# amikey/kaldi-ctc

Hardware: AMD Instinct MI355X
Metric: CTC-train frames/sec, 5×BLSTM-512 mb=16, at 1/2/4/8 MI355X; loss match (higher is better)
Workload: dtype f32

## Files before the change

include/ctc.h:

```cpp
#ifndef KALDI_CTC_AMD_CTC_H_
#define KALDI_CTC_AMD_CTC_H_

#include <stddef.h>

#ifdef __cplusplus
extern "C" {
#endif

struct ihipStream_t;
typedef struct ihipStream_t *ctcStream_t;

typedef enum {
  CTC_STATUS_SUCCESS = 0,
  CTC_STATUS_MEMOPS_FAILED = 1,
  CTC_STATUS_INVALID_VALUE = 2,
  CTC_STATUS_EXECUTION_FAILED = 3,
  CTC_STATUS_UNKNOWN_ERROR = 4
} ctcStatus_t;

typedef enum { CTC_CPU = 0, CTC_GPU = 1 } ctcComputeLocation;

struct ctcOptions {
  ctcComputeLocation loc;
  union {
// ... 11 lines not shown
                             const int *const input_lengths, int alphabet_size,
                             int minibatch, float *costs, void *workspace,
                             struct ctcOptions options);

ctcStatus_t get_workspace_size(const int *const label_lengths,
                               const int *const input_lengths, int alphabet_size,
                               int minibatch, struct ctcOptions info,
                               size_t *size_bytes);

ctcStatus_t mictc_compute_ctc_loss_async(const float *activations, float *gradients,
                                         const int *flat_labels, const int *label_lengths,
                                         const int *input_lengths, int alphabet_size,
                                         int minibatch, double *costs_dev, void *workspace,
                                         ctcStream_t stream, int blank_label);

int mictc_set_frame_group(int m);

int mictc_set_win(int on);

#ifdef __cplusplus
}
#endif
#endif
```

kaldi-ctc_amd/csrc/ctc.hip:

```cpp
#include <algorithm>
#include <cstring>
#include <type_traits>
#include <atomic>
#include <vector>

#include "common.h"
#include "ctc.h"
#include "prof.h"

namespace kctc {
namespace ctcimpl {

constexpr int kMaxLabel = 639;
constexpr int kThreads = 256;
constexpr int kABThreads = 512;
constexpr int kABWaves = kABThreads / 64;
constexpr int kSPT = (2 * kMaxLabel + 1 + kABThreads - 1) / kABThreads;
constexpr int kFR = 8;

struct UttDesc {
  int T, L, S, feasible, lab_off, pad;
  long long ab_off;
  long long off_off;
};
// ... 478 lines not shown
}

template <bool SPILL, int SPT>
__global__ __launch_bounds__(kABThreads) void ctc_alpha_beta(
    const float *__restrict__ lp, int N, int A, int blank, UttDesc *__restrict__ descs,
    const int *__restrict__ labels, float *__restrict__ spill, double *__restrict__ offs,
    double *__restrict__ costs, AbLds lay) {
  if (blockIdx.x >= (unsigned)N) ab_body<SPILL, SPT, true>(lp, N, A, blank, descs, labels, spill, offs, costs, lay);
  else ab_body<SPILL, SPT, false>(lp, N, A, blank, descs, labels, spill, offs, costs, lay);
}

__global__ __launch_bounds__(kThreads) void ctc_grad(
    const float *__restrict__ acts, const float *__restrict__ logz, float *__restrict__ grads,
    int N, int A, int T_max, int blank, const UttDesc *__restrict__ descs,
    const int *__restrict__ links, const int *__restrict__ owners, const float *__restrict__ spill,
    const double *__restrict__ offs, const double *__restrict__ costs) {
  extern __shared__ __attribute__((aligned(16))) char smem[];
  const int n = blockIdx.y, t0 = blockIdx.x * kFR, tid = threadIdx.x;
  const UttDesc d = descs[n];
  const int T = d.feasible ? d.T : 0, L = d.L, S = d.S;
  const int nf = min(kFR, T_max - t0);
  if (t0 >= T) {
    for (int it = tid; it < nf * A; it += kThreads) {
      int f = it / A, a = it - f * A;
      grads[((long)(t0 + f) * N + n) * A + a] = 0.f;
    }
    return;
  }
  float *occ = reinterpret_cast<float *>(smem);
  int *nxt = reinterpret_cast<int *>(occ + kFR * S);
  int *owner = nxt + (L > 0 ? L : 1);
  float *gblank = reinterpret_cast<float *>(owner + A);
  float *gtot = gblank + kFR;
  for (int a = tid; a < A; a += kThreads) owner[a] = owners[(long)n * A + a];
  for (int j = tid; j < L; j += kThreads) nxt[j] = links[d.lab_off + j];
  const double logp = -costs[n];
  const float *al = spill + d.ab_off;
  const float *be = al + (long long)T * S;
  const double *oa = offs + d.off_off, *ob = oa + T;
  const int nreal = min(nf, T - t0);
// ... 22 lines not shown
  __syncthreads();
  for (int it = tid; it < nf * A; it += kThreads) {
    const int f = it / A, a = it - f * A, t = t0 + f;
    const long idx = ((long)t * N + n) * A + a;
    float g = 0.f;
    if (t < T) {
      float gam = 0.f;
      if (a == blank) {
        gam = gblank[f];
      } else {
        for (int j = owner[a]; j >= 0; j = nxt[j]) gam += occ[f * S + 2 * j + 1];
        gam *= gtot[f];
      }
      g = expf(acts[idx] - logz[(long)t * N + n]) - gam;
    }
    grads[idx] = g;
  }
}

struct Staging {
  char *buf = nullptr;
  size_t cap = 0;
  hipEvent_t ev = nullptr;
  bool pending = false;
};
static thread_local Staging g_stage;

static char *staging_acquire(size_t bytes) {
  Staging &s = g_stage;
  if (s.pending) {
    if (hipEventSynchronize(s.ev) != hipSuccess) return nullptr;
// ... 18 lines not shown
static std::atomic<int> g_frame_group{0};
static int frame_group() {
  int m = g_frame_group.load(std::memory_order_relaxed);
  if (m <= 0) {
    m = 8;
    int expect = 0;
    g_frame_group.compare_exchange_strong(expect, m);
    m = g_frame_group.load(std::memory_order_relaxed);
  }
  return m;
}

static std::atomic<int> g_win{1};
static bool win_enabled() { return g_win.load(std::memory_order_relaxed) != 0; }

static ctcStatus_t launch(const float *acts, float *grads, const int *flat_labels,
                          const int *label_lengths, const int *input_lengths, int A, int N,
                          double *costs_dev, void *workspace, hipStream_t stream, int blank) {
  Layout lay;
  std::vector<UttDesc> descs;
  bool bad = false;
  if (!make_layout(label_lengths, input_lengths, A, N, &lay, &descs, &bad) || bad)
    return CTC_STATUS_INVALID_VALUE;
  if (blank < 0 || blank >= A || !acts || !workspace) return CTC_STATUS_INVALID_VALUE;
  long long nlab = 0;
  for (int n = 0; n < N; n++) nlab += label_lengths[n];
  for (long long i = 0; i < nlab; i++)
    if (flat_labels[i] < 0 || flat_labels[i] >= A || flat_labels[i] == blank)
      return CTC_STATUS_INVALID_VALUE;
  char *ws = static_cast<char *>(workspace);
  char *stage = staging_acquire(lay.costs);
  if (!stage) return CTC_STATUS_MEMOPS_FAILED;
  memcpy(stage + lay.desc, descs.data(), sizeof(UttDesc) * N);
  if (nlab) memcpy(stage + lay.labels, flat_labels, sizeof(int) * nlab);
  {
    int *links = reinterpret_cast<int *>(stage + lay.links), *owner = reinterpret_cast<int *>(stage + lay.owner);
    std::fill(owner, owner + (size_t)N * A, -1);
    long long off = 0;
    for (int n = 0; n < N; n++) {
      const int L = label_lengths[n];
      int *own = owner + (size_t)n * A;
      for (int j = L - 1; j >= 0; j--) {
        const int k = flat_labels[off + j];
        links[off + j] = own[k];
        own[k] = j;
      }
      off += L;
    }
  }
  if (hipMemcpyAsync(ws, stage, lay.costs, hipMemcpyHostToDevice, stream) != hipSuccess)
    return CTC_STATUS_MEMOPS_FAILED;
  staging_release(stream);
  UttDesc *d_desc = reinterpret_cast<UttDesc *>(ws + lay.desc);
  const int *d_lab = reinterpret_cast<const int *>(ws + lay.labels);
  float *d_logz = reinterpret_cast<float *>(ws + lay.logz);
  float *d_spill = reinterpret_cast<float *>(ws + lay.spill);
  double *d_offs = reinterpret_cast<double *>(ws + lay.offs);
  const long rows = (long)lay.T_max * N;
  float *d_lp = reinterpret_cast<float *>(ws + lay.lp);
  if (rows > 0) {
    ProfSpan ps(stream, "ctc_logz");
    hipLaunchKernelGGL(ctc_logz, dim3(ceil_div(rows, 4)), dim3(256), 0, stream, acts, A, rows,
                       d_logz, d_lp);
  }
  const int want = grads != nullptr;
  {
    int Smax = 1;
// ... 34 lines not shown
        else go(ctc_alpha_beta<false, kSPT>, N);
      }
    }
  }
  if (want && lay.T_max > 0) {
    int Lmax = 0;
    for (int n = 0; n < N; n++) Lmax = label_lengths[n] > Lmax ? label_lengths[n] : Lmax;
    const int Smax = 2 * Lmax + 1;
    size_t shm = sizeof(float) * kFR * Smax + sizeof(int) * (Lmax > 0 ? Lmax : 1) +
                 sizeof(int) * A + 2 * sizeof(float) * kFR;
    if (shm > 160 * 1024) return CTC_STATUS_INVALID_VALUE;
    ProfSpan ps(stream, "ctc_grad");
    hipLaunchKernelGGL(ctc_grad, dim3(ceil_div(lay.T_max, kFR), N), dim3(kThreads), shm, stream,
                       acts, d_logz, grads, N, A, lay.T_max, blank, d_desc,
                       reinterpret_cast<const int *>(ws + lay.links), reinterpret_cast<const int *>(ws + lay.owner),
                       d_spill, d_offs, costs_dev);
  }
  if (hipGetLastError() != hipSuccess) return CTC_STATUS_EXECUTION_FAILED;
  return CTC_STATUS_SUCCESS;
}

}
}

using namespace kctc::ctcimpl;

extern "C" {

int get_warpctc_version(void) { return 2; }

int mictc_set_frame_group(int m) {
// ... 26 lines not shown
  Layout lay;
  bool bad = false;
  if (!make_layout(label_lengths, input_lengths, alphabet_size, minibatch, &lay, nullptr, &bad) ||
      bad)
    return CTC_STATUS_INVALID_VALUE;
  *size_bytes = lay.total;
  return CTC_STATUS_SUCCESS;
}

ctcStatus_t mictc_compute_ctc_loss_async(const float *activations, float *gradients,
                                         const int *flat_labels, const int *label_lengths,
                                         const int *input_lengths, int alphabet_size,
                                         int minibatch, double *costs_dev, void *workspace,
                                         ctcStream_t stream, int blank_label) {
  if (!costs_dev) return CTC_STATUS_INVALID_VALUE;
  try {
    return launch(activations, gradients, flat_labels, label_lengths, input_lengths,
                  alphabet_size, minibatch, costs_dev, workspace,
                  reinterpret_cast<hipStream_t>(stream), blank_label);
  } catch (...) {
    return CTC_STATUS_UNKNOWN_ERROR;
  }
}

ctcStatus_t compute_ctc_loss(const float *const activations, float *gradients,
                             const int *const flat_labels, const int *const label_lengths,
                             const int *const input_lengths, int alphabet_size, int minibatch,
                             float *costs, void *workspace, struct ctcOptions options) {
  if (options.loc != CTC_GPU || !costs) return CTC_STATUS_INVALID_VALUE;
  Layout lay;
  bool bad = false;
  if (!make_layout(label_lengths, input_lengths, alphabet_size, minibatch, &lay, nullptr, &bad) ||
      bad)
    return CTC_STATUS_INVALID_VALUE;
// ... 18 lines not shown
```

kaldi-ctc_amd/csrc/elementwise.h:

```cpp
#pragma once
#include <hip/hip_runtime.h>

#include <cstddef>

namespace kctc {

void clip_sgd_update(hipStream_t s, float *w, const float *dw, long n, float lr, float clip,
                     const unsigned *skip = nullptr);
void momentum_update(hipStream_t s, float *w, float *delta, const float *dw, long n, float lr, float clip,
                     float m, const unsigned *skip = nullptr);
void rownorm_clip(hipStream_t s, float *d, long rows, int dim, float thr, int *nclipped);
void row_argmax(hipStream_t s, const float *m, long rows, int cols, int *ids);
size_t sum_rows_ws_floats(long rows, int cols);
void sum_rows(hipStream_t s, const float *X, long rows, int cols, float alpha, float beta,
              float *out, float *ws);
void fill(hipStream_t s, float *p, long n, float v);
void scale_inplace(hipStream_t s, float *p, long n, float alpha);
void axpy(hipStream_t s, float *y, const float *x, long n, float alpha);
void add_randn(hipStream_t s, float *x, long n, float stddev, unsigned long long seed);
size_t dot_ws_bytes();
void dot_f64(hipStream_t s, const float *a, const float *b, long n, double *out, void *ws);

constexpr int kMaxSplice = 32;
void splice_rows(hipStream_t s, const float *in, int dim, int ns, long rows, const int *ctx, int nctx, int first,
// ... 15 lines not shown
```

kaldi-ctc_amd/csrc/elementwise.hip:

```cpp
#include "common.h"
#include "elementwise.h"

namespace kctc {
namespace {

typedef float floatx4 __attribute__((ext_vector_type(4)));

__global__ __launch_bounds__(256) void k_clip_sgd(float *__restrict__ w, const float *__restrict__ dw,
                                                  long n, float lr, float clip, const unsigned *skip) {
  if (skip && *skip) return;
  const long n4 = n / 4;
  const long stride = (long)gridDim.x * 256;
  const bool vec = ((uintptr_t)w % 16 == 0) && ((uintptr_t)dw % 16 == 0);
  long i = (long)blockIdx.x * 256 + threadIdx.x;
  if (vec) {
    for (; i < n4; i += stride) {
      floatx4 g = reinterpret_cast<const floatx4 *>(dw)[i];
      floatx4 v = reinterpret_cast<floatx4 *>(w)[i];
#pragma unroll
      for (int j = 0; j < 4; j++) {
        float x = g[j];
        if (clip > 0.f) x = fminf(fmaxf(x, -clip), clip);
        v[j] += lr * x;
      }
      reinterpret_cast<floatx4 *>(w)[i] = v;
    }
    i = n4 * 4 + (long)blockIdx.x * 256 + threadIdx.x;
  }
  for (; i < n; i += stride) {
    float x = dw[i];
    if (clip > 0.f) x = fminf(fmaxf(x, -clip), clip);
    w[i] += lr * x;
  }
}

__global__ __launch_bounds__(256) void k_rownorm_clip(float *__restrict__ d, long rows, int dim,
                                                      float inv_thr2, int *__restrict__ nclipped) {
  const long row = (long)blockIdx.x * 4 + (threadIdx.x >> 6);
  const int lane = threadIdx.x & 63;
  __shared__ int cnt[4];
  int clipped = 0;
  if (row < rows) {
    float *r = d + row * dim;
    float ss = 0.f;
    const bool vec = (dim % 4 == 0) && ((uintptr_t)r % 16 == 0);
    if (vec) {
      for (int j = lane; j < dim / 4; j += 64) {
        floatx4 v = reinterpret_cast<const floatx4 *>(r)[j];
// ... 109 lines not shown
  }
}

void momentum_update(hipStream_t s, float *w, float *delta, const float *dw, long n, float lr, float clip,
                     float m, const unsigned *skip) {
  if (n <= 0) return;
  hipLaunchKernelGGL(k_momentum, dim3(grid_for(n)), dim3(256), 0, s, w, delta, dw, n, lr, clip, m, skip);
}

void clip_sgd_update(hipStream_t s, float *w, const float *dw, long n, float lr, float clip,
                     const unsigned *skip) {
  if (n <= 0) return;
  hipLaunchKernelGGL(k_clip_sgd, dim3(grid_for((n + 3) / 4)), dim3(256), 0, s, w, dw, n, lr, clip, skip);
}

void rownorm_clip(hipStream_t s, float *d, long rows, int dim, float thr, int *nclipped) {
  if (rows <= 0) return;
  hipLaunchKernelGGL(k_rownorm_clip, dim3(ceil_div(rows, 4)), dim3(256), 0, s, d, rows, dim,
                     1.f / (thr * thr), nclipped);
}

void row_argmax(hipStream_t s, const float *m, long rows, int cols, int *ids) {
  if (rows <= 0) return;
  hipLaunchKernelGGL(k_row_argmax, dim3(ceil_div(rows, 4)), dim3(256), 0, s, m, rows, cols, ids);
}

size_t sum_rows_ws_floats(long rows, int cols) { return (size_t)64 * cols; }

void sum_rows(hipStream_t s, const float *X, long rows, int cols, float alpha, float beta,
              float *out, float *ws) {
// ... 197 lines not shown
```

kaldi-ctc_amd/csrc/nnet.cpp:

```cpp
#include "nnet.h"
#include "kaldi_io.h"

#include <algorithm>
#include <cmath>
#include <cstdio>
#include <cstring>
#include <iomanip>
#include <iostream>
#include <sstream>

#include "common.h"
#include "ctc.h"
#include "decodable.h"
#include "dropout.h"
#include "elementwise.h"
#include "gemm.h"
#include "prof.h"

namespace kctc {
namespace nnet2 {

int levenshtein(const int *ref, int m, const int *hyp, int n) {
  if (m <= 0) return n > 0 ? n : 0;
  if (n <= 0) return m;
// ... 136 lines not shown

uint64_t Rng::next() {
  uint64_t z = (s += 0x9E3779B97F4A7C15ULL);
  z = (z ^ (z >> 30)) * 0xBF58476D1CE4E5B9ULL;
  z = (z ^ (z >> 27)) * 0x94D049BB133111EBULL;
  return z ^ (z >> 31);
}
double Rng::uniform() { return ((double)(next() >> 11) + 0.5) * (1.0 / 9007199254740992.0); }
double Rng::gauss() {
  const double u1 = uniform(), u2 = uniform();
  return std::sqrt(-2.0 * std::log(u1)) * std::cos(6.283185307179586 * u2);
}

static hipStream_t S() { return CuDevice::Instantiate().stream; }

static std::vector<std::string> split_ws(const std::string &s) {
  std::vector<std::string> out;
  std::istringstream is(s);
  std::string t;
  while (is >> t) out.push_back(t);
  return out;
}

static bool take(const std::string &name, std::string *args, std::string *val) {
  auto parts = split_ws(*args);
  const std::string ne = name + "=";
  for (size_t i = 0; i < parts.size(); i++) {
    if (parts[i].compare(0, ne.size(), ne) == 0) {
      *val = parts[i].substr(ne.size());
      std::string rest;
// ... 339 lines not shown
                                 workspace_.p, workspace_.bytes, reserve_.p, reserve_.bytes, DeviceError(),
                                 dev0.stream2, &wg);
      if (st) throw std::runtime_error("rnn_backward_data failed: " + std::to_string(st));
    }
    if (!wg.done) {
      dev0.Fork();
      ProfScope ps("layer_rnn_backward_weights", ws);
      int st = rnn_backward_weights(desc_, ws, T, N, in_value.Data(), out_value.Data(), workspace_.p,
                                    workspace_.bytes, to_update->grad_.f(), reserve_.p, reserve_.bytes,
                                    side_gemm_blocks(), input_bound_, nullptr, packed_input_cols(T, N), false,
                                    wgrad_prepack(in_value, out_value));
      if (st) throw std::runtime_error("rnn_backward_weights failed: " + std::to_string(st));
    }
    return;
  }
  {
    ProfScope ps("layer_rnn_backward_data");
    const RnnPrepack *pre = pre_.done && pre_ver_ == pver_ ? &pre_ : nullptr;
    int st = rnn_backward_data(desc_, S(), T, N, out_value.Data(), out_deriv.Data(), params_.f(),
                               in_deriv ? in_deriv->Data() : nullptr, workspace_.p, workspace_.bytes,
                               reserve_.p, reserve_.bytes, DeviceError(), CuDevice::Instantiate().stream2, nullptr,
                               pre);
    if (st) throw std::runtime_error("rnn_backward_data failed: " + std::to_string(st));
  }
  if (to_update_in) {
    auto *to_update = dynamic_cast<CuDNNRecurrentComponent *>(to_update_in);
    if (!to_update) throw std::invalid_argument("CuDNNRecurrentComponent: bad to_update");
    auto &dev = CuDevice::Instantiate();
    hipStream_t ws = dev.side ? dev.side : S();
    dev.Fork();
    to_update->grad_stream_ = ws;
    KCTC_HIP_CHECK(hipMemsetAsync(to_update->grad_.p, 0, sizeof(float) * NumParameters(), ws));
    ProfScope ps("layer_rnn_backward_weights", ws);
    int st = rnn_backward_weights(desc_, ws, T, N, in_value.Data(), out_value.Data(), workspace_.p,
                                  workspace_.bytes, to_update->grad_.f(), reserve_.p, reserve_.bytes,
                                  dev.side ? side_gemm_blocks() : 0, input_bound_,
                                  (!in_deriv && dev.side) ? dev.stream2 : nullptr, packed_input_cols(T, N),
                                  in_deriv && dev.side,
                                  wgrad_prepack(in_value, out_value));
    if (st) throw std::runtime_error("rnn_backward_weights failed: " + std::to_string(st));
  }
}

const RnnPrepack *CuDNNRecurrentComponent::wgrad_prepack(const CuMatrixBase &in_value,
                                                         const CuMatrixBase &out_value) const {
  return pre_.wdone && in_value.Data() == pre_x_ && out_value.Data() == pre_y_ ? &pre_ : nullptr;
}

bool CuDNNRecurrentComponent::PackedOutput(const void **rows, const void **cols) const {
  *rows = *cols = nullptr;
  if (!reserve_.p || seq_length_ <= 0 || mini_batch_ <= 0) return false;
  if (reserve_.bytes < sizeof(float) * (size_t)rnn_reserve_layout(desc_, seq_length_, mini_batch_).total) return false;
// ... 65 lines not shown

void UpdatableComponent::Scale(float scale) { scale_inplace(S(), ParamData(), NumParameters(), scale); }

void UpdatableComponent::Add(float alpha, const UpdatableComponent &other) {
  CheckSameKind(other, "Add");
  axpy(S(), ParamData(), const_cast<UpdatableComponent &>(other).ParamData(), NumParameters(), alpha);
}

int CuDNNRecurrentComponent::side_gemm_blocks() const {
  return 512;
}

void CuDNNRecurrentComponent::ApplyUpdate(const unsigned *skip) {
  ++pver_;
  UpdateWith(params_.f(), grad_.f(), clip_gradient_, skip);
}

Component *CuDNNRecurrentComponent::Copy() const {
  auto *c = new CuDNNRecurrentComponent;
  c->CopyUpdatableFrom(*this);
  c->desc_ = desc_;
  c->max_seq_length_ = max_seq_length_;
  c->param_stddev_ = param_stddev_;
  c->bias_stddev_ = bias_stddev_;
  c->clip_gradient_ = clip_gradient_;
  const long P = NumParameters();
  c->params_.ensure(sizeof(float) * P);
  c->grad_.ensure(sizeof(float) * P);
  KCTC_HIP_CHECK(hipMemcpyAsync(c->params_.p, params_.p, sizeof(float) * P, hipMemcpyDeviceToDevice, S()));
  return c;
// ... 505 lines not shown
    gemm_f32(S(), g);
  }
  if (to_update_in) {
    auto *to_update = dynamic_cast<AffineComponent *>(to_update_in);
    if (!to_update) throw std::invalid_argument("AffineComponent: bad to_update");
    GemmArgs g;
    g.transA = true;
    g.M = out_dim_; g.N = in_dim_; g.K = (int)rows;
    g.A = out_deriv.Data(); g.lda = out_dim_;
    g.B = in_value.Data(); g.ldb = in_dim_;
    g.C = to_update->grad_.f(); g.ldc = in_dim_;
    g.split_k = gemm_pick_split(g.M, g.N, g.K, 1);
    const size_t wsf = (size_t)g.split_k * g.M * g.N + sum_rows_ws_floats(rows, out_dim_);
    ws_.ensure(sizeof(float) * wsf);
    g.ws = ws_.f();
    gemm_f32(S(), g);
    sum_rows(S(), out_deriv.Data(), rows, out_dim_, 1.f, 0.f,
             to_update->grad_.f() + (long)in_dim_ * out_dim_, ws_.f() + (size_t)g.split_k * g.M * g.N);
  }
}

Component *AffineComponent::Copy() const {
  auto *c = new AffineComponent;
  c->CopyUpdatableFrom(*this);
  c->in_dim_ = in_dim_;
  c->out_dim_ = out_dim_;
  const long P = NumParameters();
  c->params_.ensure(sizeof(float) * P);
  c->grad_.ensure(sizeof(float) * P);
  KCTC_HIP_CHECK(hipMemcpyAsync(c->params_.p, params_.p, sizeof(float) * P, hipMemcpyDeviceToDevice, S()));
  return c;
}

void AffineComponent::ApplyUpdate(const unsigned *skip) {
  UpdateWith(params_.f(), grad_.f(), 0.f, skip);
}
void AffineComponent::Vectorize(float *host) const {
  auto v = d2h(params_.f(), NumParameters());
  std::copy(v.begin(), v.end(), host);
}
void AffineComponent::UnVectorize(const float *host) { h2d(params_.f(), host, NumParameters()); }

void AffineComponent::Write(std::ostream &os, bool binary) const {
  auto v = d2h(params_.f(), NumParameters());
  WriteToken(os, binary, "<AffineComponent>");
  WriteToken(os, binary, "<LearningRate>");
  kio::WriteFloat(os, binary, learning_rate_);
  WriteToken(os, binary, "<LinearParams>");
  kio::WriteFloatMatrix(os, binary, v.data(), out_dim_, in_dim_);
  WriteToken(os, binary, "<BiasParams>");
// ... 233 lines not shown
  const long rows = (long)T_max * N;
  set_minibatch(nnet_, N);
  err_word_.ensure(256);
  KCTC_HIP_CHECK(hipMemsetAsync(err_word_.p, 0, sizeof(unsigned), S()));
  if (inject_err_) {
    KCTC_HIP_CHECK(hipMemcpyAsync(err_word_.p, &inject_err_, sizeof(unsigned), hipMemcpyHostToDevice, S()));
    KCTC_HIP_CHECK(hipStreamSynchronize(S()));
    inject_err_ = 0;
  }
  for (int c = 0; c < C; c++)
    if (auto *r = dynamic_cast<CuDNNRecurrentComponent *>(&nnet_->GetComponent(c)))
      r->SetErrorWord(static_cast<unsigned *>(err_word_.p));
  forward_data_.resize(C + 1);
  SetupChunks(T_max, N);
  forward_data_[0].SetView(const_cast<float *>(feats), rows * nnet_->NumSplice(), nnet_->InputDim());
  Propagate(T_max, N);

  const CuMatrixBase &out = forward_data_[C];
  const int A = nnet_->OutputDim();
  for (int n = 0; n < N; n++)
    if (label_lengths[n] < 0) throw std::invalid_argument("negative label length");
  size_t ws = 0;
  {
    ctcOptions o;
    o.loc = CTC_GPU;
    o.stream = reinterpret_cast<ctcStream_t>(S());
    o.blank_label = 0;
    ctcStatus_t st = get_workspace_size(label_lengths, num_frames, A, N, o, &ws);
    if (st != CTC_STATUS_SUCCESS)
      throw std::runtime_error(std::string("get_workspace_size: ") + ctcGetStatusString(st));
    if (ws > ctc_ws_.bytes) {
      std::vector<int> worst_l(N, std::min(T_max, 639)), worst_t(N, T_max);
      size_t w2 = 0;
      if (get_workspace_size(worst_l.data(), worst_t.data(), A, N, o, &w2) == CTC_STATUS_SUCCESS)
        ws = std::max(ws, w2);
    }
  }
  ctc_ws_.ensure(ws);
  costs_dev_.ensure(sizeof(double) * N);
  ids_dev_.ensure(sizeof(int) * rows);
  CuMatrix &deriv = deriv_a_;
  deriv.Resize(rows, A);
  {
    ProfScope ps("layer_ctc");
    ctcStatus_t st = mictc_compute_ctc_loss_async(out.Data(), update_ ? deriv.Data() : nullptr,
                                                  flat_labels, label_lengths, num_frames, A, N,
                                                  static_cast<double *>(costs_dev_.p), ctc_ws_.p,
                                                  reinterpret_cast<ctcStream_t>(S()), 0);
    if (st != CTC_STATUS_SUCCESS)
      throw std::runtime_error(std::string("compute_ctc_loss: ") + ctcGetStatusString(st));
  }
  {
    ProfScope ps("argmax");
    row_argmax(S(), out.Data(), rows, A, static_cast<int *>(ids_dev_.p));
  }
  if (update_) Backprop(T_max, N);

  Slot &sl = slots_[next_];
  const size_t need = sizeof(double) * N + sizeof(int) * rows + sizeof(unsigned) * C;
  if (need > sl.bytes) {
    if (sl.pinned) {
      if (sl.ev) KCTC_HIP_CHECK(hipEventSynchronize(sl.ev));
      (void)hipHostFree(sl.pinned);
    }
    KCTC_HIP_CHECK(hipHostMalloc((void **)&sl.pinned, need, hipHostMallocDefault));
    sl.bytes = need;
  }
  if (!sl.ev) KCTC_HIP_CHECK(hipEventCreateWithFlags(&sl.ev, hipEventDisableTiming));
  double *hcost = reinterpret_cast<double *>(sl.pinned);
  int *hids = reinterpret_cast<int *>(sl.pinned + sizeof(double) * N);
  unsigned *herr = reinterpret_cast<unsigned *>(hids + rows);
// ... 106 lines not shown
      continue;
    }
    out.Resize((long)T * N, comp.OutputDim());
    const auto *rnn = dynamic_cast<const CuDNNRecurrentComponent *>(&comp);
    const CuDNNRecurrentComponent *next = nullptr;
    if (rnn) {
      int c2 = c + 1;
      while (c2 < C && nnet_->GetComponent(c2).IsIdentityForward()) c2++;
      if (c2 < C) next = dynamic_cast<const CuDNNRecurrentComponent *>(&nnet_->GetComponent(c2));
    }
    if (next) rnn->PropagateChained(in, &out, *next);
    else comp.Propagate(chunk_info_[c], chunk_info_[c + 1], in, &out);
  }
}

void NnetCtcUpdater::Backprop(int T, int N) {
  const int C = nnet_->NumComponents();
  const long rows = (long)T * N;
  const int A = nnet_->OutputDim();
  {
    ProfScope ps("scale");
    scale_inplace(S(), deriv_a_.Data(), rows * (long)A, -1.f);
  }
  CuMatrix *cur = &deriv_a_, *other = &deriv_b_;
  const int first = nnet_->FirstUpdatableComponent();
  int max_dim = A;
  for (int c = 0; c <= C; c++) max_dim = std::max(max_dim, chunk_info_[c].feat_dim);
  std::vector<int> updated;
  for (int c = C - 1; c >= first; c--) {
    Component &comp = nnet_->GetComponent(c);
    const CuMatrixBase &in = forward_data_[c], &outv = forward_data_[c + 1];
    Component *to_update = &comp;
    const bool need_in_deriv = c > first;
    CuMatrixBase *in_deriv = nullptr;
    CuMatrixBase view;
    if (need_in_deriv) {
      if (comp.IsIdentityForward()) {
        view = CuMatrixBase(cur->Data(), rows, comp.InputDim());
        in_deriv = &view;
// ... 5 lines not shown
    }
    if (auto *cg = dynamic_cast<ClipGradientComponent *>(&comp)) {
      cg->rng_ = &repair_rng_;
      if (cg->Shadow()) to_update = cg->Shadow();
    }
    const CuMatrixBase od(cur->Data(), rows, comp.OutputDim());
    const bool rec = exchange_ && dynamic_cast<CuDNNRecurrentComponent *>(&comp);
    if (rec) exchange_->BeforeRecurrence(S());
    comp.Backprop(chunk_info_[c], chunk_info_[c + 1], in, outv, od, to_update, in_deriv);
    if (rec) exchange_->AfterRecurrence();
    if (comp.IsUpdatable()) {
      auto *u = static_cast<UpdatableComponent *>(&comp);
      if (exchange_) exchange_->GradReady(c, u->GradData(), u->NumParameters(), u->GradStream());
      updated.push_back(c);
    }
    if (need_in_deriv && !comp.IsIdentityForward()) std::swap(cur, other);
  }
  CuDevice::Instantiate().Join();
  if (exchange_) exchange_->Finish();
  if (exchange_ && exchange_->WorldSize() > 1 && err_word_.p) {
    unsigned *err = static_cast<unsigned *>(err_word_.p);
    err_flag_.ensure(256);
    err_word_to_flag(S(), err, err_flag_.f());
    exchange_->AllReduceSum(err_flag_.f(), 1, S());
    flag_to_err_word(S(), err_flag_.f(), err);
  }
  for (int c : updated) {
    ProfScope ps("update");
    static_cast<UpdatableComponent *>(&nnet_->GetComponent(c))->ApplyUpdate(err_word_.p ? static_cast<const unsigned *>(err_word_.p) : nullptr);
  }
}

}
}
```

kaldi-ctc_amd/csrc/nnet.h:

```cpp
#pragma once
#include <hip/hip_runtime.h>

#include <cstdint>
#include <iosfwd>
#include <map>
#include <memory>
#include <string>
#include <utility>
#include <vector>

#include "clipgrad.h"
#include "glibc_rand.h"
#include "rnn.h"

namespace kctc {
namespace nnet2 {

struct DevBuf {
  void *p = nullptr;
  size_t bytes = 0;
  DevBuf() = default;
  DevBuf(const DevBuf &) = delete;
  DevBuf &operator=(const DevBuf &) = delete;
  DevBuf(DevBuf &&o) noexcept : p(o.p), bytes(o.bytes) { o.p = nullptr; o.bytes = 0; }
  DevBuf &operator=(DevBuf &&o) noexcept {
    std::swap(p, o.p);
// ... 31 lines not shown

struct ChunkInfo {
  int feat_dim = 0, num_chunks = 0, chunk_size = 0;
  int first_offset = 0;
  long NumRows() const { return (long)num_chunks * chunk_size; }
  int NumCols() const { return feat_dim; }
  int NumChunks() const { return num_chunks; }
};

struct CuDevice {
  int device = 0;
  hipStream_t stream = nullptr;
  hipStream_t side = nullptr;
  hipStream_t stream2 = nullptr;
  hipEvent_t fork_ev = nullptr, join_ev = nullptr;
  void Fork();
  void Join();
  bool profiling = false;
  struct Span { std::string family; hipEvent_t a, b; hipStream_t s; };
  std::vector<Span> spans;
  std::vector<size_t> open;
  std::vector<hipEvent_t> pool;
  std::map<std::string, std::pair<double, int>> prof;
  void Begin(const char *family, hipStream_t s = nullptr);
  void End();
  void Collect();
  static CuDevice &Instantiate();
};

struct Rng {
// ... 39 lines not shown
  virtual void SetZero(bool treat_as_gradient);
  virtual double DotProduct(const UpdatableComponent &other) const;
  virtual void PerturbParams(float stddev);
  virtual void Scale(float scale);
  virtual void Add(float alpha, const UpdatableComponent &other);
  bool IsGradient() const { return is_gradient_; }
  static void SetPerturbSeed(unsigned long long seed);
  virtual long NumParameters() const = 0;
  virtual void Vectorize(float *host) const = 0;
  virtual void UnVectorize(const float *host) = 0;
  virtual float *GradData() = 0;
  virtual float *ParamData() = 0;
  hipStream_t GradStream() const;
  void ResetGradStream() { grad_stream_ = nullptr; }
  virtual void ApplyUpdate(const unsigned *skip = nullptr) = 0;
  void SetMomentum(float m);
  float Momentum() const { return momentum_; }

 protected:
  void UpdateWith(float *params, const float *grad, float clip, const unsigned *skip);
  void CopyUpdatableFrom(const UpdatableComponent &o);
  void CheckSameKind(const UpdatableComponent &o, const char *what) const;
  float learning_rate_ = 0.001f;
  bool is_gradient_ = false;
  hipStream_t grad_stream_ = nullptr;
  float momentum_ = 0.f;
  DevBuf delta_;
};

class SpliceComponent : public Component {
// ... 36 lines not shown
                const CuMatrixBase &out_deriv, Component *to_update,
                CuMatrixBase *in_deriv) const override;
  void Write(std::ostream &os, bool binary) const override;
  void Read(std::istream &is, bool binary) override;
  Component *Copy() const override;
  void SetZero(bool treat_as_gradient) override;
  long NumParameters() const override { return desc_.params_size(); }
  void Vectorize(float *host) const override;
  void UnVectorize(const float *host) override;
  float *GradData() override { return grad_.f(); }
  float *ParamData() override {
    ++pver_;
    return params_.f();
  }
  void ApplyUpdate(const unsigned *skip = nullptr) override;
  void SetPrepackDx(bool on) const { prepack_dx_ = on; }
  void SetPrepackW(bool on) const { prepack_w_ = on; }
  unsigned *DeviceError() const { return err_ext_ ? err_ext_ : err_; }
  void SetErrorWord(unsigned *e) const { err_ext_ = e; }
  int side_gemm_blocks() const;
  const RnnPrepack *wgrad_prepack(const CuMatrixBase &in_value, const CuMatrixBase &out_value) const;
  const RnnDesc &Desc() const { return desc_; }
  void SetPrecision(int prec) {
    if (prec == 1 && desc_.mode != kLstm && desc_.mode != kGru)
      throw std::invalid_argument("bf16 products exist for LSTM / GRU only");
    rnn_set_precision(desc_, prec);
  }
  void SetMiniBatch(int n) const { mini_batch_ = n; }
  bool PropagatedShape(int T, int N) const { return seq_length_ == T && mini_batch_ == N && reserve_.p; }
  void PropagateChained(const CuMatrixBase &in, CuMatrixBase *out, const CuDNNRecurrentComponent &next) const;
// ... 143 lines not shown
  bool BackpropNeedsOutput() const override { return false; }
  void Propagate(const ChunkInfo &, const ChunkInfo &, const CuMatrixBase &in,
                 CuMatrixBase *out) const override;
  void Backprop(const ChunkInfo &, const ChunkInfo &, const CuMatrixBase &in_value,
                const CuMatrixBase &, const CuMatrixBase &out_deriv, Component *to_update,
                CuMatrixBase *in_deriv) const override;
  void Write(std::ostream &os, bool binary) const override;
  void Read(std::istream &is, bool binary) override;
  Component *Copy() const override;
  long NumParameters() const override { return (long)(in_dim_ + 1) * out_dim_; }
  void Vectorize(float *host) const override;
  void UnVectorize(const float *host) override;
  float *GradData() override { return grad_.f(); }
  float *ParamData() override { return params_.f(); }
  void ApplyUpdate(const unsigned *skip = nullptr) override;

 private:
  int in_dim_ = 0, out_dim_ = 0;
  DevBuf params_, grad_;
  mutable DevBuf ws_;
};

class Nnet {
 public:
  ~Nnet();
  void Init(const std::string &config, Rng &rng);
  int NumComponents() const { return (int)components_.size(); }
  Component &GetComponent(int c) { return *components_[c]; }
  const Component &GetComponent(int c) const { return *components_[c]; }
  int FirstUpdatableComponent() const;
  int LastUpdatableComponent() const;
  void SetComponent(int c, Component *component);
  int LeftContext() const;
  int RightContext() const;
  int NumSplice() const { return 1 + LeftContext() + RightContext(); }
// ... 41 lines not shown
  int Pending() const { return pending_; }
  MinibatchStats Finish();
  void SetExchange(GradExchange *ex) { exchange_ = ex; }
  const CuMatrixBase &Forward(const float *feats, int T_max, int N);
  const std::vector<int> &LastBestPath() const { return last_ids_; }
  const std::vector<double> &LastCosts() const { return last_costs_; }
  const CuMatrixBase &Output() const { return forward_data_.empty() ? empty_ : forward_data_.back(); }
  void Srand(unsigned seed) { repair_rng_.Seed(seed); }
  long RandCalls() const { return repair_rng_.Calls(); }
  void InjectStepError(unsigned word) { inject_err_ = word; }
  void ComponentsChanged();

 private:
  void SetupChunks(int T_max, int N);
  void Propagate(int T, int N);
  void Backprop(int T, int N);
  Nnet *nnet_;
  bool update_;
  GradExchange *exchange_ = nullptr;
  GlibcRand repair_rng_{0};
  std::vector<CuMatrix> forward_data_;
  std::vector<int> last_ids_;
  std::vector<double> last_costs_;
  CuMatrixBase empty_;
  std::vector<ChunkInfo> chunk_info_;
  CuMatrix deriv_a_, deriv_b_;
  DevBuf ctc_ws_, costs_dev_, ids_dev_;
  DevBuf err_word_;
  DevBuf err_flag_;
  unsigned inject_err_ = 0;
  struct Slot {
    char *pinned = nullptr;
    size_t bytes = 0;
    hipEvent_t ev = nullptr;
    int N = 0, nerr = 0;
    long rows = 0;
    std::vector<int> num_frames, labels, label_lengths;
  };
  Slot slots_[2];
  int next_ = 0, pending_ = 0;
};
// ... 4 lines not shown
```

Baseline: 863,500.

## Overlap CTC prep, argmax and top-layer wgrad on side streams; fuse SGD updates

Splits CTC into a prepare step (label upload, layout), which now runs on a side stream during forward propagation, and a run step that folds the gradient negation into the gradient kernel, so the separate scale pass goes away. Argmax and the top affine layer's weight-gradient GEMM move to the side stream. The last RNN layer's grad memset moves onto stream2 before backward-data. All SGD updates are batched into a single multi-segment kernel launch. Each path is gated by an environment variable that defaults to on. The cost is more cross-stream events, an extra deriv buffer, and more complex buffer ping-pong logic.

```diff
diff --git a/include/ctc.h b/include/ctc.h
--- a/include/ctc.h
+++ b/include/ctc.h
@@ -49,6 +49,14 @@
                                          int minibatch, double *costs_dev, void *workspace,
                                          ctcStream_t stream, int blank_label);
 
+ctcStatus_t mictc_ctc_prepare_async(const int *flat_labels, const int *label_lengths,
+                                    const int *input_lengths, int alphabet_size, int minibatch,
+                                    void *workspace, ctcStream_t stream, int blank_label);
+ctcStatus_t mictc_ctc_run_async(const float *activations, float *gradients, const int *label_lengths,
+                                const int *input_lengths, int alphabet_size, int minibatch,
+                                double *costs_dev, void *workspace, ctcStream_t stream, int blank_label,
+                                int negate_gradients);
+
 int mictc_set_frame_group(int m);
 
 int mictc_set_win(int on);
diff --git a/kaldi-ctc_amd/csrc/ctc.hip b/kaldi-ctc_amd/csrc/ctc.hip
--- a/kaldi-ctc_amd/csrc/ctc.hip
+++ b/kaldi-ctc_amd/csrc/ctc.hip
@@ -516,7 +516,7 @@
     const float *__restrict__ acts, const float *__restrict__ logz, float *__restrict__ grads,
     int N, int A, int T_max, int blank, const UttDesc *__restrict__ descs,
     const int *__restrict__ links, const int *__restrict__ owners, const float *__restrict__ spill,
-    const double *__restrict__ offs, const double *__restrict__ costs) {
+    const double *__restrict__ offs, const double *__restrict__ costs, float gscale) {
   extern __shared__ __attribute__((aligned(16))) char smem[];
   const int n = blockIdx.y, t0 = blockIdx.x * kFR, tid = threadIdx.x;
   const UttDesc d = descs[n];
@@ -525,7 +525,7 @@
   if (t0 >= T) {
     for (int it = tid; it < nf * A; it += kThreads) {
       int f = it / A, a = it - f * A;
-      grads[((long)(t0 + f) * N + n) * A + a] = 0.f;
+      grads[((long)(t0 + f) * N + n) * A + a] = 0.f * gscale;
     }
     return;
   }
@@ -578,7 +578,7 @@
       }
       g = expf(acts[idx] - logz[(long)t * N + n]) - gam;
     }
-    grads[idx] = g;
+    grads[idx] = g * gscale;
   }
 }
 
@@ -627,15 +627,14 @@
 static std::atomic<int> g_win{1};
 static bool win_enabled() { return g_win.load(std::memory_order_relaxed) != 0; }
 
-static ctcStatus_t launch(const float *acts, float *grads, const int *flat_labels,
-                          const int *label_lengths, const int *input_lengths, int A, int N,
-                          double *costs_dev, void *workspace, hipStream_t stream, int blank) {
+static ctcStatus_t prepare(const int *flat_labels, const int *label_lengths, const int *input_lengths, int A,
+                           int N, void *workspace, hipStream_t stream, int blank) {
   Layout lay;
   std::vector<UttDesc> descs;
   bool bad = false;
   if (!make_layout(label_lengths, input_lengths, A, N, &lay, &descs, &bad) || bad)
     return CTC_STATUS_INVALID_VALUE;
-  if (blank < 0 || blank >= A || !acts || !workspace) return CTC_STATUS_INVALID_VALUE;
+  if (blank < 0 || blank >= A || !workspace) return CTC_STATUS_INVALID_VALUE;
   long long nlab = 0;
   for (int n = 0; n < N; n++) nlab += label_lengths[n];
   for (long long i = 0; i < nlab; i++)
@@ -664,6 +663,18 @@
   if (hipMemcpyAsync(ws, stage, lay.costs, hipMemcpyHostToDevice, stream) != hipSuccess)
     return CTC_STATUS_MEMOPS_FAILED;
   staging_release(stream);
+  return CTC_STATUS_SUCCESS;
+}
+
+static ctcStatus_t run(const float *acts, float *grads, const int *label_lengths, const int *input_lengths,
+                       int A, int N, double *costs_dev, void *workspace, hipStream_t stream, int blank,
+                       float gscale) {
+  Layout lay;
+  bool bad = false;
+  if (!make_layout(label_lengths, input_lengths, A, N, &lay, nullptr, &bad) || bad)
+    return CTC_STATUS_INVALID_VALUE;
+  if (blank < 0 || blank >= A || !acts || !workspace) return CTC_STATUS_INVALID_VALUE;
+  char *ws = static_cast<char *>(workspace);
   UttDesc *d_desc = reinterpret_cast<UttDesc *>(ws + lay.desc);
   const int *d_lab = reinterpret_cast<const int *>(ws + lay.labels);
   float *d_logz = reinterpret_cast<float *>(ws + lay.logz);
@@ -728,7 +739,7 @@
     hipLaunchKernelGGL(ctc_grad, dim3(ceil_div(lay.T_max, kFR), N), dim3(kThreads), shm, stream,
                        acts, d_logz, grads, N, A, lay.T_max, blank, d_desc,
                        reinterpret_cast<const int *>(ws + lay.links), reinterpret_cast<const int *>(ws + lay.owner),
-                       d_spill, d_offs, costs_dev);
+                       d_spill, d_offs, costs_dev, gscale);
   }
   if (hipGetLastError() != hipSuccess) return CTC_STATUS_EXECUTION_FAILED;
   return CTC_STATUS_SUCCESS;
@@ -785,10 +796,38 @@
                                          int minibatch, double *costs_dev, void *workspace,
                                          ctcStream_t stream, int blank_label) {
   if (!costs_dev) return CTC_STATUS_INVALID_VALUE;
+  if (!activations) return CTC_STATUS_INVALID_VALUE;
   try {
-    return launch(activations, gradients, flat_labels, label_lengths, input_lengths,
-                  alphabet_size, minibatch, costs_dev, workspace,
-                  reinterpret_cast<hipStream_t>(stream), blank_label);
+    hipStream_t s = reinterpret_cast<hipStream_t>(stream);
+    ctcStatus_t st = prepare(flat_labels, label_lengths, input_lengths, alphabet_size, minibatch, workspace, s,
+                             blank_label);
+    if (st != CTC_STATUS_SUCCESS) return st;
+    return run(activations, gradients, label_lengths, input_lengths, alphabet_size, minibatch, costs_dev,
+               workspace, s, blank_label, 1.f);
+  } catch (...) {
+    return CTC_STATUS_UNKNOWN_ERROR;
+  }
+}
+
+ctcStatus_t mictc_ctc_prepare_async(const int *flat_labels, const int *label_lengths,
+                                    const int *input_lengths, int alphabet_size, int minibatch,
+                                    void *workspace, ctcStream_t stream, int blank_label) {
+  try {
+    return prepare(flat_labels, label_lengths, input_lengths, alphabet_size, minibatch, workspace,
+                   reinterpret_cast<hipStream_t>(stream), blank_label);
+  } catch (...) {
+    return CTC_STATUS_UNKNOWN_ERROR;
+  }
+}
+
+ctcStatus_t mictc_ctc_run_async(const float *activations, float *gradients, const int *label_lengths,
+                                const int *input_lengths, int alphabet_size, int minibatch,
+                                double *costs_dev, void *workspace, ctcStream_t stream, int blank_label,
+                                int negate_gradients) {
+  if (!costs_dev) return CTC_STATUS_INVALID_VALUE;
+  try {
+    return run(activations, gradients, label_lengths, input_lengths, alphabet_size, minibatch, costs_dev,
+               workspace, reinterpret_cast<hipStream_t>(stream), blank_label, negate_gradients ? -1.f : 1.f);
   } catch (...) {
     return CTC_STATUS_UNKNOWN_ERROR;
   }
diff --git a/kaldi-ctc_amd/csrc/elementwise.h b/kaldi-ctc_amd/csrc/elementwise.h
--- a/kaldi-ctc_amd/csrc/elementwise.h
+++ b/kaldi-ctc_amd/csrc/elementwise.h
@@ -7,6 +7,18 @@
 
 void clip_sgd_update(hipStream_t s, float *w, const float *dw, long n, float lr, float clip,
                      const unsigned *skip = nullptr);
+constexpr int kMaxClipSgdSegs = 16;
+struct ClipSgdSeg {
+  float *w;
+  const float *dw;
+  long n;
+  float lr, clip;
+};
+struct ClipSgdSegs {
+  ClipSgdSeg seg[kMaxClipSgdSegs];
+  int count = 0;
+};
+void clip_sgd_update_multi(hipStream_t s, const ClipSgdSegs &segs, const unsigned *skip = nullptr);
 void momentum_update(hipStream_t s, float *w, float *delta, const float *dw, long n, float lr, float clip,
                      float m, const unsigned *skip = nullptr);
 void rownorm_clip(hipStream_t s, float *d, long rows, int dim, float thr, int *nclipped);
diff --git a/kaldi-ctc_amd/csrc/elementwise.hip b/kaldi-ctc_amd/csrc/elementwise.hip
--- a/kaldi-ctc_amd/csrc/elementwise.hip
+++ b/kaldi-ctc_amd/csrc/elementwise.hip
@@ -6,13 +6,12 @@
 
 typedef float floatx4 __attribute__((ext_vector_type(4)));
 
-__global__ __launch_bounds__(256) void k_clip_sgd(float *__restrict__ w, const float *__restrict__ dw,
-                                                  long n, float lr, float clip, const unsigned *skip) {
-  if (skip && *skip) return;
+__device__ __forceinline__ void clip_sgd_body(float *__restrict__ w, const float *__restrict__ dw, long n, float lr,
+                                              float clip, long bid, long nblk) {
   const long n4 = n / 4;
-  const long stride = (long)gridDim.x * 256;
+  const long stride = nblk * 256;
   const bool vec = ((uintptr_t)w % 16 == 0) && ((uintptr_t)dw % 16 == 0);
-  long i = (long)blockIdx.x * 256 + threadIdx.x;
+  long i = bid * 256 + threadIdx.x;
   if (vec) {
     for (; i < n4; i += stride) {
       floatx4 g = reinterpret_cast<const floatx4 *>(dw)[i];
@@ -25,13 +24,25 @@
       }
       reinterpret_cast<floatx4 *>(w)[i] = v;
     }
-    i = n4 * 4 + (long)blockIdx.x * 256 + threadIdx.x;
+    i = n4 * 4 + bid * 256 + threadIdx.x;
   }
   for (; i < n; i += stride) {
     float x = dw[i];
     if (clip > 0.f) x = fminf(fmaxf(x, -clip), clip);
     w[i] += lr * x;
   }
+}
+
+__global__ __launch_bounds__(256) void k_clip_sgd(float *__restrict__ w, const float *__restrict__ dw,
+                                                  long n, float lr, float clip, const unsigned *skip) {
+  if (skip && *skip) return;
+  clip_sgd_body(w, dw, n, lr, clip, blockIdx.x, gridDim.x);
+}
+
+__global__ __launch_bounds__(256) void k_clip_sgd_multi(ClipSgdSegs segs, const unsigned *skip) {
+  if (skip && *skip) return;
+  const ClipSgdSeg &sg = segs.seg[blockIdx.y];
+  clip_sgd_body(sg.w, sg.dw, sg.n, sg.lr, sg.clip, blockIdx.x, gridDim.x);
 }
 
 __global__ __launch_bounds__(256) void k_rownorm_clip(float *__restrict__ d, long rows, int dim,
@@ -171,6 +182,14 @@
   hipLaunchKernelGGL(k_clip_sgd, dim3(grid_for((n + 3) / 4)), dim3(256), 0, s, w, dw, n, lr, clip, skip);
 }
 
+void clip_sgd_update_multi(hipStream_t s, const ClipSgdSegs &segs, const unsigned *skip) {
+  if (segs.count <= 0) return;
+  if (segs.count > kMaxClipSgdSegs) throw std::invalid_argument("clip_sgd_update_multi: too many segments");
+  int gx = 1;
+  for (int i = 0; i < segs.count; i++) gx = std::max(gx, grid_for((segs.seg[i].n + 3) / 4));
+  hipLaunchKernelGGL(k_clip_sgd_multi, dim3(gx, segs.count), dim3(256), 0, s, segs, skip);
+}
+
 void rownorm_clip(hipStream_t s, float *d, long rows, int dim, float thr, int *nclipped) {
   if (rows <= 0) return;
   hipLaunchKernelGGL(k_rownorm_clip, dim3(ceil_div(rows, 4)), dim3(256), 0, s, d, rows, dim,
diff --git a/kaldi-ctc_amd/csrc/nnet.cpp b/kaldi-ctc_amd/csrc/nnet.cpp
--- a/kaldi-ctc_amd/csrc/nnet.cpp
+++ b/kaldi-ctc_amd/csrc/nnet.cpp
@@ -174,6 +174,11 @@
 
 static hipStream_t S() { return CuDevice::Instantiate().stream; }
 
+static bool env_on(const char *name) {
+  const char *e = getenv(name);
+  return !e || atoi(e) != 0;
+}
+
 static std::vector<std::string> split_ws(const std::string &s) {
   std::vector<std::string> out;
   std::istringstream is(s);
@@ -543,6 +548,16 @@
     }
     return;
   }
+  const bool tail = to_update_in && !in_deriv && dev0.side && dev0.stream2 && env_on("KCTC_TAIL_COMPUTE");
+  if (tail) {
+    auto *to_update = dynamic_cast<CuDNNRecurrentComponent *>(to_update_in);
+    if (!to_update) throw std::invalid_argument("CuDNNRecurrentComponent: bad to_update");
+    dev0.Fork();
+    KCTC_HIP_CHECK(hipStreamWaitEvent(dev0.stream2, dev0.fork_ev, 0));
+    KCTC_HIP_CHECK(hipMemsetAsync(to_update->grad_.p, 0, sizeof(float) * NumParameters(), dev0.stream2));
+    if (!dev0.tail_ev) KCTC_HIP_CHECK(hipEventCreateWithFlags(&dev0.tail_ev, hipEventDisableTiming));
+    KCTC_HIP_CHECK(hipEventRecord(dev0.tail_ev, dev0.stream2));
+  }
   {
     ProfScope ps("layer_rnn_backward_data");
     const RnnPrepack *pre = pre_.done && pre_ver_ == pver_ ? &pre_ : nullptr;
@@ -557,14 +572,20 @@
     if (!to_update) throw std::invalid_argument("CuDNNRecurrentComponent: bad to_update");
     auto &dev = CuDevice::Instantiate();
     hipStream_t ws = dev.side ? dev.side : S();
-    dev.Fork();
-    to_update->grad_stream_ = ws;
-    KCTC_HIP_CHECK(hipMemsetAsync(to_update->grad_.p, 0, sizeof(float) * NumParameters(), ws));
+    hipStream_t s2 = (!in_deriv && dev.side) ? dev.stream2 : nullptr;
+    if (tail) {
+      ws = S();
+      to_update->grad_stream_ = nullptr;
+      KCTC_HIP_CHECK(hipStreamWaitEvent(ws, dev.tail_ev, 0));
+    } else {
+      dev.Fork();
+      to_update->grad_stream_ = ws;
+      KCTC_HIP_CHECK(hipMemsetAsync(to_update->grad_.p, 0, sizeof(float) * NumParameters(), ws));
+    }
     ProfScope ps("layer_rnn_backward_weights", ws);
     int st = rnn_backward_weights(desc_, ws, T, N, in_value.Data(), out_value.Data(), workspace_.p,
                                   workspace_.bytes, to_update->grad_.f(), reserve_.p, reserve_.bytes,
-                                  dev.side ? side_gemm_blocks() : 0, input_bound_,
-                                  (!in_deriv && dev.side) ? dev.stream2 : nullptr, packed_input_cols(T, N),
+                                  dev.side ? side_gemm_blocks() : 0, input_bound_, s2, packed_input_cols(T, N),
                                   in_deriv && dev.side,
                                   wgrad_prepack(in_value, out_value));
     if (st) throw std::runtime_error("rnn_backward_weights failed: " + std::to_string(st));
@@ -660,6 +681,13 @@
 void CuDNNRecurrentComponent::ApplyUpdate(const unsigned *skip) {
   ++pver_;
   UpdateWith(params_.f(), grad_.f(), clip_gradient_, skip);
+}
+
+bool CuDNNRecurrentComponent::UpdateSegment(ClipSgdSeg *seg) {
+  if (momentum_ != 0.f) return false;
+  ++pver_;
+  *seg = ClipSgdSeg{params_.f(), grad_.f(), NumParameters(), learning_rate_, clip_gradient_};
+  return true;
 }
 
 Component *CuDNNRecurrentComponent::Copy() const {
@@ -1195,8 +1223,16 @@
     const size_t wsf = (size_t)g.split_k * g.M * g.N + sum_rows_ws_floats(rows, out_dim_);
     ws_.ensure(sizeof(float) * wsf);
     g.ws = ws_.f();
-    gemm_f32(S(), g);
-    sum_rows(S(), out_deriv.Data(), rows, out_dim_, 1.f, 0.f,
+    auto &dev = CuDevice::Instantiate();
+    hipStream_t ws = side_wgrad_ && dev.side ? dev.side : S();
+    if (ws != S()) {
+      dev.Fork();
+      to_update->grad_stream_ = ws;
+    } else {
+      to_update->grad_stream_ = nullptr;
+    }
+    gemm_f32(ws, g);
+    sum_rows(ws, out_deriv.Data(), rows, out_dim_, 1.f, 0.f,
              to_update->grad_.f() + (long)in_dim_ * out_dim_, ws_.f() + (size_t)g.split_k * g.M * g.N);
   }
 }
@@ -1215,6 +1251,11 @@
 
 void AffineComponent::ApplyUpdate(const unsigned *skip) {
   UpdateWith(params_.f(), grad_.f(), 0.f, skip);
+}
+bool AffineComponent::UpdateSegment(ClipSgdSeg *seg) {
+  if (momentum_ != 0.f) return false;
+  *seg = ClipSgdSeg{params_.f(), grad_.f(), NumParameters(), learning_rate_, 0.f};
+  return true;
 }
 void AffineComponent::Vectorize(float *host) const {
   auto v = d2h(params_.f(), NumParameters());
@@ -1478,14 +1519,13 @@
   forward_data_.resize(C + 1);
   SetupChunks(T_max, N);
   forward_data_[0].SetView(const_cast<float *>(feats), rows * nnet_->NumSplice(), nnet_->InputDim());
-  Propagate(T_max, N);
-
-  const CuMatrixBase &out = forward_data_[C];
   const int A = nnet_->OutputDim();
   for (int n = 0; n < N; n++)
     if (label_lengths[n] < 0) throw std::invalid_argument("negative label length");
-  size_t ws = 0;
-  {
+  auto &dev = CuDevice::Instantiate();
+  const bool top_side = dev.side && env_on("KCTC_TOP_SIDE");
+  auto ctc_ws_size = [&]() {
+    size_t ws = 0;
     ctcOptions o;
     o.loc = CTC_GPU;
     o.stream = reinterpret_cast<ctcStream_t>(S());
@@ -1499,26 +1539,56 @@
       if (get_workspace_size(worst_l.data(), worst_t.data(), A, N, o, &w2) == CTC_STATUS_SUCCESS)
         ws = std::max(ws, w2);
     }
-  }
-  ctc_ws_.ensure(ws);
+    ctc_ws_.ensure(ws);
+  };
+  if (top_side) {
+    ctc_ws_size();
+    dev.Fork();
+    ctcStatus_t st = mictc_ctc_prepare_async(flat_labels, label_lengths, num_frames, A, N, ctc_ws_.p,
+                                             reinterpret_cast<ctcStream_t>(dev.side), 0);
+    if (st != CTC_STATUS_SUCCESS)
+      throw std::runtime_error(std::string("compute_ctc_loss: ") + ctcGetStatusString(st));
+    if (!ctc_prep_ev_) KCTC_HIP_CHECK(hipEventCreateWithFlags(&ctc_prep_ev_, hipEventDisableTiming));
+    KCTC_HIP_CHECK(hipEventRecord(ctc_prep_ev_, dev.side));
+  }
+  Propagate(T_max, N);
+
+  const CuMatrixBase &out = forward_data_[C];
+  if (!top_side) ctc_ws_size();
   costs_dev_.ensure(sizeof(double) * N);
   ids_dev_.ensure(sizeof(int) * rows);
-  CuMatrix &deriv = deriv_a_;
+  CuMatrix &deriv = top_side ? deriv_ctc_ : deriv_a_;
   deriv.Resize(rows, A);
+  if (top_side) {
+    dev.Fork();
+    ProfScope ps("argmax", dev.side);
+    row_argmax(dev.side, out.Data(), rows, A, static_cast<int *>(ids_dev_.p));
+  }
   {
     ProfScope ps("layer_ctc");
-    ctcStatus_t st = mictc_compute_ctc_loss_async(out.Data(), update_ ? deriv.Data() : nullptr,
-                                                  flat_labels, label_lengths, num_frames, A, N,
-                                                  static_cast<double *>(costs_dev_.p), ctc_ws_.p,
-                                                  reinterpret_cast<ctcStream_t>(S()), 0);
+    ctcStatus_t st;
+    if (top_side) {
+      KCTC_HIP_CHECK(hipStreamWaitEvent(S(), ctc_prep_ev_, 0));
+      st = mictc_ctc_run_async(out.Data(), update_ ? deriv.Data() : nullptr, label_lengths, num_frames, A, N,
+                               static_cast<double *>(costs_dev_.p), ctc_ws_.p,
+                               reinterpret_cast<ctcStream_t>(S()), 0, 1);
+    } else {
+      st = mictc_compute_ctc_loss_async(out.Data(), update_ ? deriv.Data() : nullptr, flat_labels,
+                                        label_lengths, num_frames, A, N, static_cast<double *>(costs_dev_.p),
+                                        ctc_ws_.p, reinterpret_cast<ctcStream_t>(S()), 0);
+    }
     if (st != CTC_STATUS_SUCCESS)
       throw std::runtime_error(std::string("compute_ctc_loss: ") + ctcGetStatusString(st));
   }
-  {
+  if (!top_side) {
     ProfScope ps("argmax");
     row_argmax(S(), out.Data(), rows, A, static_cast<int *>(ids_dev_.p));
   }
-  if (update_) Backprop(T_max, N);
+  auto *top_affine = top_side ? dynamic_cast<AffineComponent *>(&nnet_->GetComponent(C - 1)) : nullptr;
+  if (top_affine) top_affine->SetSideWgrad(true);
+  if (update_) Backprop(T_max, N, &deriv, top_side);
+  else if (top_side) dev.Join();
+  if (top_affine) top_affine->SetSideWgrad(false);
 
   Slot &sl = slots_[next_];
   const size_t need = sizeof(double) * N + sizeof(int) * rows + sizeof(unsigned) * C;
@@ -1655,15 +1725,15 @@
   }
 }
 
-void NnetCtcUpdater::Backprop(int T, int N) {
+void NnetCtcUpdater::Backprop(int T, int N, CuMatrix *deriv, bool negated) {
   const int C = nnet_->NumComponents();
   const long rows = (long)T * N;
   const int A = nnet_->OutputDim();
-  {
+  if (!negated) {
     ProfScope ps("scale");
-    scale_inplace(S(), deriv_a_.Data(), rows * (long)A, -1.f);
-  }
-  CuMatrix *cur = &deriv_a_, *other = &deriv_b_;
+    scale_inplace(S(), deriv->Data(), rows * (long)A, -1.f);
+  }
+  CuMatrix *cur = deriv, *other = deriv == &deriv_a_ ? &deriv_b_ : &deriv_a_;
   const int first = nnet_->FirstUpdatableComponent();
   int max_dim = A;
   for (int c = 0; c <= C; c++) max_dim = std::max(max_dim, chunk_info_[c].feat_dim);
@@ -1699,7 +1769,10 @@
       if (exchange_) exchange_->GradReady(c, u->GradData(), u->NumParameters(), u->GradStream());
       updated.push_back(c);
     }
-    if (need_in_deriv && !comp.IsIdentityForward()) std::swap(cur, other);
+    if (need_in_deriv && !comp.IsIdentityForward()) {
+      std::swap(cur, other);
+      if (other != &deriv_a_ && other != &deriv_b_) other = cur == &deriv_a_ ? &deriv_b_ : &deriv_a_;
+    }
   }
   CuDevice::Instantiate().Join();
   if (exchange_) exchange_->Finish();
@@ -1710,11 +1783,26 @@
     exchange_->AllReduceSum(err_flag_.f(), 1, S());
     flag_to_err_word(S(), err_flag_.f(), err);
   }
+  const unsigned *skip = err_word_.p ? static_cast<const unsigned *>(err_word_.p) : nullptr;
+  bool fused = env_on("KCTC_FUSED_UPDATE") && (int)updated.size() <= kMaxClipSgdSegs;
+  for (int c : updated)
+    if (static_cast<UpdatableComponent *>(&nnet_->GetComponent(c))->Momentum() != 0.f) fused = false;
+  if (fused) {
+    ProfScope ps("update");
+    ClipSgdSegs segs;
+    for (int c : updated) {
+      ClipSgdSeg sg;
+      static_cast<UpdatableComponent *>(&nnet_->GetComponent(c))->UpdateSegment(&sg);
+      if (sg.n > 0) segs.seg[segs.count++] = sg;
+    }
+    clip_sgd_update_multi(S(), segs, skip);
+    return;
+  }
   for (int c : updated) {
     ProfScope ps("update");
-    static_cast<UpdatableComponent *>(&nnet_->GetComponent(c))->ApplyUpdate(err_word_.p ? static_cast<const unsigned *>(err_word_.p) : nullptr);
-  }
-}
-
-}
-}
+    static_cast<UpdatableComponent *>(&nnet_->GetComponent(c))->ApplyUpdate(skip);
+  }
+}
+
+}
+}
diff --git a/kaldi-ctc_amd/csrc/nnet.h b/kaldi-ctc_amd/csrc/nnet.h
--- a/kaldi-ctc_amd/csrc/nnet.h
+++ b/kaldi-ctc_amd/csrc/nnet.h
@@ -10,6 +10,7 @@
 #include <vector>
 
 #include "clipgrad.h"
+#include "elementwise.h"
 #include "glibc_rand.h"
 #include "rnn.h"
 
@@ -71,6 +72,7 @@
   hipStream_t side = nullptr;
   hipStream_t stream2 = nullptr;
   hipEvent_t fork_ev = nullptr, join_ev = nullptr;
+  hipEvent_t tail_ev = nullptr;
   void Fork();
   void Join();
   bool profiling = false;
@@ -140,6 +142,7 @@
   hipStream_t GradStream() const;
   void ResetGradStream() { grad_stream_ = nullptr; }
   virtual void ApplyUpdate(const unsigned *skip = nullptr) = 0;
+  virtual bool UpdateSegment(ClipSgdSeg *seg) = 0;
   void SetMomentum(float m);
   float Momentum() const { return momentum_; }
 
@@ -206,6 +209,7 @@
     return params_.f();
   }
   void ApplyUpdate(const unsigned *skip = nullptr) override;
+  bool UpdateSegment(ClipSgdSeg *seg) override;
   void SetPrepackDx(bool on) const { prepack_dx_ = on; }
   void SetPrepackW(bool on) const { prepack_w_ = on; }
   unsigned *DeviceError() const { return err_ext_ ? err_ext_ : err_; }
@@ -379,11 +383,14 @@
   float *GradData() override { return grad_.f(); }
   float *ParamData() override { return params_.f(); }
   void ApplyUpdate(const unsigned *skip = nullptr) override;
+  bool UpdateSegment(ClipSgdSeg *seg) override;
+  void SetSideWgrad(bool on) const { side_wgrad_ = on; }
 
  private:
   int in_dim_ = 0, out_dim_ = 0;
   DevBuf params_, grad_;
   mutable DevBuf ws_;
+  mutable bool side_wgrad_ = false;
 };
 
 class Nnet {
@@ -455,7 +462,7 @@
  private:
   void SetupChunks(int T_max, int N);
   void Propagate(int T, int N);
-  void Backprop(int T, int N);
+  void Backprop(int T, int N, CuMatrix *deriv, bool negated);
   Nnet *nnet_;
   bool update_;
   GradExchange *exchange_ = nullptr;
@@ -466,6 +473,8 @@
   CuMatrixBase empty_;
   std::vector<ChunkInfo> chunk_info_;
   CuMatrix deriv_a_, deriv_b_;
+  CuMatrix deriv_ctc_;
+  hipEvent_t ctc_prep_ev_ = nullptr;
   DevBuf ctc_ws_, costs_dev_, ids_dev_;
   DevBuf err_word_;
   DevBuf err_flag_;
```

Measured after the change: 866,900 (median of 6 runs). About the same (+0.4%).
